# farhad-dalirani/StereoVision-SLAM

Hardware: AMD Instinct MI355X
Metric: stereo frames/sec (track + local BA), KITTI-00-shaped synthetic stereo 1241x376 (620x188 after the reference's 1/2 decimation) (higher is better)
Workload: dtype u8/i32 fixed-point (pyramid, LK), f32 (GFTT), f64 (LM, BA)

## Files before the change

stereovision-slam_amd/csrc/k_lk.h:

```cpp
#pragma once
#include "dev_common.h"

struct LkJob { int prev_slot, next_slot, pt_ofs, npts; };
struct LkParams {
    int max_level;
    int max_count;
    double eps2;
    double min_eig_thr;
    int use_initial_flow;
    float eig_num_thr;
    int eig_use_div;
    int njobs, blocks_per_job;
};

#define LK_WIN 11
#define LK_NPIX 121
#define LK_W_BITS 14
#define LK_REG 32
#ifndef LK_WAVES_PER_BLOCK
#define LK_WAVES_PER_BLOCK 1
#endif
#define LK_IROW 20

typedef uint32_t lk_u32_ua __attribute__((aligned(1)));
typedef uint16_t lk_u16_ua __attribute__((aligned(1)));
typedef short lk_s2 __attribute__((ext_vector_type(2)));

__device__ __forceinline__ int lk_dot2(uint32_t a, uint32_t b, int c)
{
    int r;
    asm("v_dot2_i32_i16 %0, %1, %2, %3" : "=v"(r) : "v"(a), "v"(b), "v"(c));
    return r;
}
#define LK_PAIR_SEL0 0x0c010c00u
__device__ __forceinline__ uint32_t lk_pair_sel(int a) { return LK_PAIR_SEL0 + (uint32_t)(a & 3) * 0x00010001u; }
__device__ __forceinline__ uint32_t lk_pair_at(const uint32_t *base32, int a, uint32_t sel)
{
    const uint32_t *q = base32 + (a >> 2);
    return __builtin_amdgcn_perm(q[1], q[0], sel);
}

__device__ __forceinline__ int lk_floor_i(float x)
{
    int r;
    asm("v_cvt_flr_i32_f32 %0, %1" : "=v"(r) : "v"(x));
    return r;
}

struct LkW { uint32_t top, bot; };

__device__ __forceinline__ LkW lk_weights(float a, float b)
{
    typedef float lk_f2 __attribute__((ext_vector_type(2)));
    const float S = (float)(1 << LK_W_BITS), M = 12582912.f;
    const float A = a * S, An = S - A, bn = 1.f - b;
    const lk_f2 p0 = (lk_f2){An, A} * (lk_f2){bn, bn} + (lk_f2){M, M};
    const uint32_t b00 = __float_as_uint(p0.x), b01 = __float_as_uint(p0.y), b10 = __float_as_uint(An * b + M);
    const uint32_t w11 = ((1u << LK_W_BITS) + 3u * 0x4B400000u) - (b00 + b01 + b10);
    LkW w;
    w.top = __builtin_amdgcn_perm(b01, b00, 0x05040100u);
    w.bot = __builtin_amdgcn_perm(w11, b10, 0x05040100u);
    return w;
}

__device__ __forceinline__ int lk_sample_u8(const uint32_t *base32, int a, int row_stride, LkW w)
{
    const uint32_t sel = lk_pair_sel(a);
    const uint32_t *q = base32 + (a >> 2);
    const int rs = row_stride >> 2;
    const uint32_t t = __builtin_amdgcn_perm(q[1], q[0], sel), b = __builtin_amdgcn_perm(q[rs + 1], q[rs], sel);
    return lk_dot2(t, w.top, lk_dot2(b, w.bot, 1 << (LK_W_BITS - 5 - 1))) >> (LK_W_BITS - 5);
}

__device__ __forceinline__ int lk_sample_diff(const uint32_t *base32, int a, int row_stride, LkW w, int acc0)
{
    const uint32_t sel = lk_pair_sel(a);
    const uint32_t *q = base32 + (a >> 2);
    const int rs = row_stride >> 2;
    const uint32_t t = __builtin_amdgcn_perm(q[1], q[0], sel), b = __builtin_amdgcn_perm(q[rs + 1], q[rs], sel);
    return lk_dot2(t, w.top, lk_dot2(b, w.bot, acc0)) >> (LK_W_BITS - 5);
}

typedef const __attribute__((address_space(3))) uint32_t *lk_lds_u32;
__device__ __forceinline__ int lk_sample_diff_at(uint32_t addr, LkW w, int acc0)
{
    lk_lds_u32 q = (lk_lds_u32)(uintptr_t)addr;
    const uint32_t t = q[0], b = q[LK_REG];
    return lk_dot2(t, w.top, lk_dot2(b, w.bot, acc0)) >> (LK_W_BITS - 5);
}

struct LkJRegs { uint32_t v[4]; };
__device__ __forceinline__ LkJRegs lk_stage_J_issue(const uint8_t *J0, uint32_t lofs, int pitch, int w, int h,
                                                    int cx, int cy, int lane, int &rx0, int &ry0)
{
    rx0 = __builtin_amdgcn_readfirstlane((cx - 10) & ~3);
    ry0 = __builtin_amdgcn_readfirstlane(cy - 10);
    const int r = lane >> 3, c4 = lane & 7;
    LkJRegs o;
    if (rx0 >= -SVS_BORDER && rx0 + LK_REG <= w + SVS_BORDER && ry0 >= -SVS_BORDER && ry0 + LK_REG <= h + SVS_BORDER) {
        const uint32_t p = lofs + (uint32_t)((ry0 + r) * pitch + (rx0 + c4 * 4));
#pragma unroll
        for (int k = 0; k < 4; ++k)
            o.v[k] = *reinterpret_cast<const uint32_t *>(J0 + (p + (uint32_t)(8 * k * pitch)));
    } else {
        const int gxmax = (w + SVS_BORDER - 4) & ~3;
        const int gx = max(-SVS_BORDER, min(rx0 + c4 * 4, gxmax));
#pragma unroll
        for (int k = 0; k < 4; ++k) {
            const int gy = max(-SVS_BORDER, min(ry0 + r + 8 * k, h + SVS_BORDER - 1));
            o.v[k] = *reinterpret_cast<const uint32_t *>(J0 + (lofs + (uint32_t)(gy * pitch + gx)));
        }
    }
    return o;
}
__device__ __forceinline__ void lk_stage_J_commit(uint32_t *sJ, const LkJRegs &o, int lane)
{
    typedef uint32_t lk_u4 __attribute__((ext_vector_type(4)));
    const int r = lane >> 3, c4 = lane & 7;
#pragma unroll
    for (int k = 0; k < 4; ++k) {
        const uint32_t cur = o.v[k];
        const uint32_t nxt = (uint32_t)__builtin_amdgcn_update_dpp(0, (int)cur, 0x101 , 0xf, 0xf, true);
        lk_u4 pr;
        pr.x = __builtin_amdgcn_perm(nxt, cur, 0x0c010c00u);
        pr.y = __builtin_amdgcn_perm(nxt, cur, 0x0c020c01u);
        pr.z = __builtin_amdgcn_perm(nxt, cur, 0x0c030c02u);
        pr.w = __builtin_amdgcn_perm(nxt, cur, 0x0c040c03u);
        *reinterpret_cast<lk_u4 *>(sJ + (r + 8 * k) * LK_REG + 4 * c4) = pr;
    }
    __builtin_amdgcn_fence(__ATOMIC_RELEASE, "wavefront");
    __builtin_amdgcn_wave_barrier();
}
__device__ __forceinline__ void lk_stage_J(uint32_t *sJ, const uint8_t *J0, uint32_t lofs, int pitch, int w, int h,
                                           int cx, int cy, int lane, int &rx0, int &ry0)
{
    const LkJRegs o = lk_stage_J_issue(J0, lofs, pitch, w, h, cx, cy, lane, rx0, ry0);
    lk_stage_J_commit(sJ, o, lane);
}

__device__ __forceinline__ float lk_sum_to_f32(long long s, float scale)
{
    const int lo = (int)s;
    const bool fits = (long long)lo == s;
    const int t = fits ? lo : (int)((s >> 1) | (s & 1));
    const uint32_t kb = fits ? __float_as_uint(scale) : __float_as_uint(2.f * scale);
    return (float)t * __uint_as_float(kb);
}

typedef unsigned lk_u2 __attribute__((ext_vector_type(2)));
__device__ __forceinline__ int lk_row_reduce(int w)
{
    w += dpp_i32<SVS_DPP_XOR1>(w);
    w += dpp_i32<SVS_DPP_XOR2>(w);
    w += dpp_i32<SVS_DPP_HALF_MIRROR>(w);
    w += dpp_i32<SVS_DPP_MIRROR>(w);
    return w;
}
__device__ __forceinline__ void lk_wave_sum2_i32(int a, int b, int &sa, int &sb)
{
    const lk_u2 r = __builtin_amdgcn_permlane16_swap((unsigned)a, (unsigned)b, false, false);
    const int v = (int)(r.x + r.y);
    const int w = lk_row_reduce(v);
    sa = __builtin_amdgcn_readlane(w, 0) + __builtin_amdgcn_readlane(w, 32);
    sb = __builtin_amdgcn_readlane(w, 16) + __builtin_amdgcn_readlane(w, 48);
}
__device__ __forceinline__ void lk_wave_sum4_i32(int a, int b, int c, int d, int &sa, int &sb, int &sc, int &sd)
{
    const lk_u2 r1 = __builtin_amdgcn_permlane16_swap((unsigned)a, (unsigned)b, false, false);
    const lk_u2 r2 = __builtin_amdgcn_permlane16_swap((unsigned)c, (unsigned)d, false, false);
    const int v1 = (int)(r1.x + r1.y), v2 = (int)(r2.x + r2.y);
    const lk_u2 q = __builtin_amdgcn_permlane32_swap((unsigned)v1, (unsigned)v2, false, false);
    const int w = lk_row_reduce((int)(q.x + q.y));
    sa = __builtin_amdgcn_readlane(w, 0);
    sb = __builtin_amdgcn_readlane(w, 16);
    sc = __builtin_amdgcn_readlane(w, 32);
    sd = __builtin_amdgcn_readlane(w, 48);
}

#ifndef LK_OCC_TEST
#define LK_OCC_TEST 0
#endif
#if LK_OCC_TEST == 1
#define LK_OCC_ATTR __attribute__((amdgpu_waves_per_eu(8, 8)))
#else
#define LK_OCC_ATTR
#endif
__global__ void __launch_bounds__(64 * LK_WAVES_PER_BLOCK) LK_OCC_ATTR
k_lk(const LkJob *jobs, const uint8_t *pyr, PyrGeom g, const float2 *prev_xy, float2 *next_xy,
     uint8_t *status, float *err, LkParams prm)
{
    __shared__ uint32_t sI_all[LK_WAVES_PER_BLOCK][16 * LK_IROW / 4 + 2];
    __shared__ uint32_t sD_all[LK_WAVES_PER_BLOCK][144];
    __shared__ __attribute__((aligned(16))) uint32_t sJ_all[LK_WAVES_PER_BLOCK][LK_REG * LK_REG];

#if LK_OCC_TEST == 2
    __shared__ uint32_t sPad[8192];
    sPad[threadIdx.x] = threadIdx.x;
    if (prm.max_count < 0) status[0] = (uint8_t)sPad[(threadIdx.x * 37) & 8191];
#endif
    const int wave = threadIdx.x >> 6, lane = threadIdx.x & 63;
    const int slot = blockIdx.x >> 3, round = slot / prm.blocks_per_job;
    const int job = round * 8 + (blockIdx.x & 7);
    if (job >= prm.njobs) return;
    const LkJob jb = jobs[job];
    const int pi = (slot - round * prm.blocks_per_job) * LK_WAVES_PER_BLOCK + wave;
    if (pi >= jb.npts) return;
    const int pt = jb.pt_ofs + pi;
    uint32_t *sI32 = sI_all[wave];
    uint32_t *sD = sD_all[wave];
    uint32_t *sJ = sJ_all[wave];

    const uint8_t *slotI = pyr + (size_t)jb.prev_slot * g.slot_bytes;
    const uint8_t *slotJ = pyr + (size_t)jb.next_slot * g.slot_bytes;

    const float2 prevp = prev_xy[pt];
    float2 nextp = next_xy[pt];
    bool st = true;
    float errv = 0.f;

    const int p0 = lane, p1 = lane + 64;
    const bool has1 = p1 < LK_NPIX;
    const int wy0 = p0 / LK_WIN, wx0 = p0 - wy0 * LK_WIN;
    const int wy1 = has1 ? p1 / LK_WIN : 0, wx1 = has1 ? p1 - wy1 * LK_WIN : 0;
    const int oI0 = (wy0 + 1) * LK_IROW + wx0 + 1, oI1 = (wy1 + 1) * LK_IROW + wx1 + 1;
    const int oD0 = wy0 * 12 + wx0, oD1 = wy1 * 12 + wx1;
    const int oJ0 = wy0 * LK_REG + wx0, oJ1 = wy1 * LK_REG + wx1;
    const uint32_t aJ0 = (uint32_t)(uintptr_t)(__attribute__((address_space(3))) uint32_t *)sJ + 4u * (uint32_t)oJ0,
                   aJ1 = (uint32_t)(uintptr_t)(__attribute__((address_space(3))) uint32_t *)sJ + 4u * (uint32_t)oJ1;
    const int sr = lane >> 2, sc = (lane & 3) * 3;
    const float FLT_SCALE = 1.f / (float)(1 << 20);
    const float e_lo = (float)(prm.eps2 * (1.0 - 2e-6)), e_hi = (float)(prm.eps2 * (1.0 + 2e-6));

    int max_level = prm.max_level;
    if (max_level > g.nlevels - 1) max_level = g.nlevels - 1;

    for (int level = max_level; level >= 0; --level) {
        const int w = g.w[level], h = g.h[level], pitch = g.pitch[level];
        const uint32_t lofs = (uint32_t)g.ofs[level] + (uint32_t)(SVS_BORDER * pitch + SVS_BORDER);
        const float lscale = __uint_as_float((uint32_t)(127 - level) << 23);
        float px = prevp.x * lscale, py = prevp.y * lscale;
        float nx, ny;
        if (level == max_level) {
            if (prm.use_initial_flow) { nx = nextp.x * lscale; ny = nextp.y * lscale; }
            else { nx = px; ny = py; }
        } else { nx = nextp.x * 2.f; ny = nextp.y * 2.f; }
        nextp.x = nx; nextp.y = ny;

        px -= 5.f; py -= 5.f;
        const int ipx = __builtin_amdgcn_readfirstlane(lk_floor_i(px)), ipy = __builtin_amdgcn_readfirstlane(lk_floor_i(py));
        const uint32_t wext = (uint32_t)(w + LK_WIN), hext = (uint32_t)(h + LK_WIN);
        if ((uint32_t)(ipx + LK_WIN) >= wext || (uint32_t)(ipy + LK_WIN) >= hext) {
            if (level == 0) { st = false; errv = 0.f; }
            continue;
        }
        const LkW iw = lk_weights(px - (float)ipx, py - (float)ipy);

        const int xs = (ipx - 1) & ~3, a0 = (ipx - 1) & 3;
        __builtin_amdgcn_wave_barrier();
        nx -= 5.f; ny -= 5.f;
        int rx0, ry0;
        LkJRegs jr;
        {
            const uint32_t ib = lofs + (uint32_t)((ipy - 1) * pitch + xs);
            const uint32_t v0 = *reinterpret_cast<const uint32_t *>(slotI + (ib + (uint32_t)((lane >> 2) * pitch + (lane & 3) * 4)));
            const uint32_t v1 = *reinterpret_cast<const uint32_t *>(slotI + (ib + (uint32_t)((lane & 15) * pitch + 16)));
            jr = lk_stage_J_issue(slotJ, lofs, pitch, w, h, lk_floor_i(nx), lk_floor_i(ny), lane, rx0, ry0);
            sI32[(lane >> 2) * (LK_IROW / 4) + (lane & 3)] = v0;
            sI32[(lane & 15) * (LK_IROW / 4) + 4] = v1;
        }
        __builtin_amdgcn_fence(__ATOMIC_RELEASE, "wavefront");
        __builtin_amdgcn_wave_barrier();
        if (lane < 48) {
            const int ab = sr * LK_IROW + a0 + sc;
            const int k8 = (ab & 3) * 8;
            const uint32_t *q = sI32 + (ab >> 2);
            const uint32_t al = q[0], ah = q[1], bl = q[LK_IROW / 4], bh = q[LK_IROW / 4 + 1],
                           cl = q[2 * (LK_IROW / 4)], ch = q[2 * (LK_IROW / 4) + 1];
            const uint32_t a4 = __builtin_amdgcn_alignbyte(ah, al, ab & 3), b4 = __builtin_amdgcn_alignbyte(bh, bl, ab & 3),
                           c4 = __builtin_amdgcn_alignbyte(ch, cl, ab & 3);
            auto pr = [](uint32_t v) -> lk_s2 { return __builtin_bit_cast(lk_s2, v); };
            const lk_s2 A01 = pr(__builtin_amdgcn_perm(0u, a4, 0x0c010c00u)), A23 = pr(__builtin_amdgcn_perm(0u, a4, 0x0c030c02u)), A4 = pr((ah >> k8) & 0xffu);
            const lk_s2 B01 = pr(__builtin_amdgcn_perm(0u, b4, 0x0c010c00u)), B23 = pr(__builtin_amdgcn_perm(0u, b4, 0x0c030c02u)), B4 = pr((bh >> k8) & 0xffu);
            const lk_s2 C01 = pr(__builtin_amdgcn_perm(0u, c4, 0x0c010c00u)), C23 = pr(__builtin_amdgcn_perm(0u, c4, 0x0c030c02u)), C4 = pr((ch >> k8) & 0xffu);
            const lk_s2 k3 = { 3, 3 }, k10 = { 10, 10 };
            const lk_s2 T001 = (A01 + C01) * k3 + B01 * k10, T023 = (A23 + C23) * k3 + B23 * k10, T04 = (A4 + C4) * k3 + B4 * k10;
            const lk_s2 T101 = C01 - A01, T123 = C23 - A23, T14 = C4 - A4;
            const lk_s2 DX01 = T023 - T001, DX2 = T04 - T023;
            const lk_s2 M01 = pr(__builtin_amdgcn_alignbyte(__builtin_bit_cast(uint32_t, T123), __builtin_bit_cast(uint32_t, T101), 2));
            const lk_s2 M2 = pr(__builtin_amdgcn_alignbyte(__builtin_bit_cast(uint32_t, T14), __builtin_bit_cast(uint32_t, T123), 2));
            const lk_s2 DY01 = (T123 + T101) * k3 + M01 * k10, DY2 = (T14 + T123) * k3 + M2 * k10;
            const uint32_t dx01 = __builtin_bit_cast(uint32_t, DX01), dy01 = __builtin_bit_cast(uint32_t, DY01);
            const uint32_t o0 = __builtin_amdgcn_perm(dy01, dx01, 0x05040100u), o1 = __builtin_amdgcn_perm(dy01, dx01, 0x07060302u),
                           o2 = __builtin_amdgcn_perm(__builtin_bit_cast(uint32_t, DY2), __builtin_bit_cast(uint32_t, DX2), 0x05040100u);
            const bool rowin = (uint32_t)(ipy + sr) < (uint32_t)h;
            sD[sr * 12 + sc + 0] = o0 & (0u - (uint32_t)(rowin & ((uint32_t)(ipx + sc + 0) < (uint32_t)w)));
            sD[sr * 12 + sc + 1] = o1 & (0u - (uint32_t)(rowin & ((uint32_t)(ipx + sc + 1) < (uint32_t)w)));
            sD[sr * 12 + sc + 2] = o2 & (0u - (uint32_t)(rowin & ((uint32_t)(ipx + sc + 2) < (uint32_t)w)));
        }
        __builtin_amdgcn_fence(__ATOMIC_RELEASE, "wavefront");
        __builtin_amdgcn_wave_barrier();
        int iv0, ix0, iy0, iv1, ix1, iy1;
        {
            iv0 = lk_sample_u8(sI32, oI0 + a0, LK_IROW, iw);
            const uint32_t d00 = sD[oD0], d01 = sD[oD0 + 1], d10 = sD[oD0 + 12], d11 = sD[oD0 + 13];
            ix0 = lk_dot2(__builtin_amdgcn_perm(d01, d00, 0x05040100u), iw.top,
                          lk_dot2(__builtin_amdgcn_perm(d11, d10, 0x05040100u), iw.bot, 1 << (LK_W_BITS - 1))) >> LK_W_BITS;
            iy0 = lk_dot2(__builtin_amdgcn_perm(d01, d00, 0x07060302u), iw.top,
                          lk_dot2(__builtin_amdgcn_perm(d11, d10, 0x07060302u), iw.bot, 1 << (LK_W_BITS - 1))) >> LK_W_BITS;
        }
        {
            iv1 = lk_sample_u8(sI32, oI1 + a0, LK_IROW, iw);
            const uint32_t d00 = sD[oD1], d01 = sD[oD1 + 1], d10 = sD[oD1 + 12], d11 = sD[oD1 + 13];
            ix1 = lk_dot2(__builtin_amdgcn_perm(d01, d00, 0x05040100u), iw.top,
                          lk_dot2(__builtin_amdgcn_perm(d11, d10, 0x05040100u), iw.bot, 1 << (LK_W_BITS - 1))) >> LK_W_BITS;
            iy1 = lk_dot2(__builtin_amdgcn_perm(d01, d00, 0x07060302u), iw.top,
                          lk_dot2(__builtin_amdgcn_perm(d11, d10, 0x07060302u), iw.bot, 1 << (LK_W_BITS - 1))) >> LK_W_BITS;
            if (!has1) { ix1 = 0; iy1 = 0; }
        }
        int sA11, sA12, sA22, sIdle;
        lk_wave_sum4_i32(__mul24(ix0, ix0) + __mul24(ix1, ix1), __mul24(ix0, iy0) + __mul24(ix1, iy1), __mul24(iy0, iy0) + __mul24(iy1, iy1), 0,
                         sA11, sA12, sA22, sIdle);
        const float A11 = (float)sA11 * FLT_SCALE, A12 = (float)sA12 * FLT_SCALE, A22 = (float)sA22 * FLT_SCALE;
        float D = A11 * A22 - A12 * A12;
        const float dd = A11 - A22;
        const float q2 = dd * dd + 4.f * A12 * A12;
        float eigNum;
        if (prm.eig_use_div) eigNum = A22 + A11 - sqrtf(q2);
        else {
            const float sq = __builtin_amdgcn_sqrtf(q2);
            eigNum = A22 + A11 - sq;
            if (fabsf(eigNum - prm.eig_num_thr) <= sq * 4.8e-7f + 1e-30f) eigNum = A22 + A11 - sqrtf(q2);
        }
        const bool eigSmall = prm.eig_use_div ? (double)(eigNum / (float)(2 * LK_WIN * LK_WIN)) < prm.min_eig_thr : eigNum < prm.eig_num_thr;
        if (eigSmall || D < 1.1920928955078125e-07f) {
            if (level == 0) st = false;
            continue;
        }
        D = 1.f / D;
        const bool narrow = sA11 <= 570000000 && sA22 <= 570000000;
        const int acc00 = (1 << (LK_W_BITS - 5 - 1)) - (iv0 << (LK_W_BITS - 5)), acc01 = (1 << (LK_W_BITS - 5 - 1)) - (iv1 << (LK_W_BITS - 5));
        const uint32_t ixx = __builtin_amdgcn_perm((uint32_t)ix1, (uint32_t)ix0, 0x05040100u), iyy = __builtin_amdgcn_perm((uint32_t)iy1, (uint32_t)iy0, 0x05040100u);
        float pdx = 0.f, pdy = 0.f, dx = 0.f, dy = 0.f;
        const float Ds = D * FLT_SCALE;
        bool moved = false, osc = false;
        lk_stage_J_commit(sJ, jr, lane);

        for (int j = 0; j < prm.max_count; ++j) {
            const int inx = __builtin_amdgcn_readfirstlane(lk_floor_i(nx)), iny = __builtin_amdgcn_readfirstlane(lk_floor_i(ny));
            if ((uint32_t)(inx + LK_WIN) >= wext || (uint32_t)(iny + LK_WIN) >= hext) {
                if (level == 0) st = false;
                break;
            }
            int ox = inx - rx0, oy = iny - ry0;
            if ((uint32_t)ox > LK_REG - 12 || (uint32_t)oy > LK_REG - 12) {
                lk_stage_J(sJ, slotJ, lofs, pitch, w, h, inx, iny, lane, rx0, ry0);
                ox = inx - rx0; oy = iny - ry0;
            }
            const LkW jw = lk_weights(nx - (float)inx, ny - (float)iny);
            const uint32_t jo = 4u * (uint32_t)(oy * LK_REG + ox);
            const int d0 = lk_sample_diff_at(aJ0 + jo, jw, acc00);
            const int d1 = lk_sample_diff_at(aJ1 + jo, jw, acc01);
            const uint32_t dd01 = __builtin_amdgcn_perm((uint32_t)d1, (uint32_t)d0, 0x05040100u);
            const int pb1 = lk_dot2(dd01, ixx, 0), pb2 = lk_dot2(dd01, iyy, 0);
            float b1, b2;
            if (narrow) {
                int s1, s2;
                lk_wave_sum2_i32(pb1, pb2, s1, s2);
                b1 = (float)s1; b2 = (float)s2;
            } else {
                b1 = lk_sum_to_f32(wave_sum_i32_wide(pb1), 1.f); b2 = lk_sum_to_f32(wave_sum_i32_wide(pb2), 1.f);
            }
            dx = (A12 * b2 - A22 * b1) * Ds;
            dy = (A12 * b1 - A11 * b2) * Ds;
            nx += dx; ny += dy;
            moved = true;
            const float dd2 = dx * dx + dy * dy;
            if (dd2 < e_lo) break;
            if (dd2 <= e_hi && (double)dx * (double)dx + (double)dy * (double)dy <= prm.eps2) break;
            if (j > 0 && fabsf(dx + pdx) <= 0.01f && fabsf(dy + pdy) <= 0.01f) {
                osc = true;
                break;
            }
            pdx = dx; pdy = dy;
        }
        if (moved) {
            nextp.x = nx + 5.f; nextp.y = ny + 5.f;
            if (osc) { nextp.x -= dx * 0.5f; nextp.y -= dy * 0.5f; }
        }

        if (st && level == 0) {
            const float fx = nextp.x - 5.f, fy = nextp.y - 5.f;
            const int inx = __builtin_amdgcn_readfirstlane(lk_floor_i(fx)), iny = __builtin_amdgcn_readfirstlane(lk_floor_i(fy));
            if (inx < -LK_WIN || inx >= w || iny < -LK_WIN || iny >= h) {
                st = false;
                continue;
            }
            int ox = inx - rx0, oy = iny - ry0;
            if (ox < 0 || ox > LK_REG - 12 || oy < 0 || oy > LK_REG - 12) {
                lk_stage_J(sJ, slotJ, lofs, pitch, w, h, inx, iny, lane, rx0, ry0);
                ox = inx - rx0; oy = iny - ry0;
            }
            const LkW jw = lk_weights(fx - (float)inx, fy - (float)iny);
            const uint32_t jo = 4u * (uint32_t)(oy * LK_REG + ox);
            const int d0 = lk_sample_diff_at(aJ0 + jo, jw, 1 << (LK_W_BITS - 5 - 1)) - iv0;
            const int d1 = lk_sample_diff_at(aJ1 + jo, jw, 1 << (LK_W_BITS - 5 - 1)) - iv1;
            const int e = (d0 < 0 ? -d0 : d0) + (has1 ? (d1 < 0 ? -d1 : d1) : 0);
            const int serr = wave_sum_i32(e);
            errv = (float)serr * 1.f / (float)(32 * LK_WIN * LK_WIN);
        }
    }
    if (lane == 0) {
        next_xy[pt] = nextp;
        status[pt] = st ? 1 : 0;
        if (err) err[pt] = errv;
    }
}
```

Measured before the change: 588,400.

## Compute all pyramid levels' LK template setup in parallel, one 16-lane row per level

The per-level template setup (I-window load, Scharr gradients, bilinear sampling, structure-tensor reduction) that used to run serially at each pyramid level inside the coarse-to-fine loop is now done once up front. Each 16-lane row of the wave handles one level. The results are handed over through LDS that aliases the J region, plus registers for the coarse levels, and the iteration loop just reads them. This removes the serial global-load latency and barriers paid at every level. In exchange it uses more registers, does 4x redundant lane work per row, and ties the code to SVS_LEVELS==4.

```diff
diff --git a/stereovision-slam_amd/csrc/k_lk.h b/stereovision-slam_amd/csrc/k_lk.h
--- a/stereovision-slam_amd/csrc/k_lk.h
+++ b/stereovision-slam_amd/csrc/k_lk.h
@@ -21,6 +21,9 @@
 #define LK_WAVES_PER_BLOCK 1
 #endif
 #define LK_IROW 20
+#define LK_SI_DW (16 * LK_IROW / 4 + 2)
+#define LK_SETUP_DW (LK_SI_DW + 144)
+#define LK_SCAL_DW 8
 
 typedef uint32_t lk_u32_ua __attribute__((aligned(1)));
 typedef uint16_t lk_u16_ua __attribute__((aligned(1)));
@@ -164,17 +167,9 @@
     sa = __builtin_amdgcn_readlane(w, 0) + __builtin_amdgcn_readlane(w, 32);
     sb = __builtin_amdgcn_readlane(w, 16) + __builtin_amdgcn_readlane(w, 48);
 }
-__device__ __forceinline__ void lk_wave_sum4_i32(int a, int b, int c, int d, int &sa, int &sb, int &sc, int &sd)
-{
-    const lk_u2 r1 = __builtin_amdgcn_permlane16_swap((unsigned)a, (unsigned)b, false, false);
-    const lk_u2 r2 = __builtin_amdgcn_permlane16_swap((unsigned)c, (unsigned)d, false, false);
-    const int v1 = (int)(r1.x + r1.y), v2 = (int)(r2.x + r2.y);
-    const lk_u2 q = __builtin_amdgcn_permlane32_swap((unsigned)v1, (unsigned)v2, false, false);
-    const int w = lk_row_reduce((int)(q.x + q.y));
-    sa = __builtin_amdgcn_readlane(w, 0);
-    sb = __builtin_amdgcn_readlane(w, 16);
-    sc = __builtin_amdgcn_readlane(w, 32);
-    sd = __builtin_amdgcn_readlane(w, 48);
+__device__ __forceinline__ float lk_uniform_f32(uint32_t v)
+{
+    return __uint_as_float((uint32_t)__builtin_amdgcn_readfirstlane((int)v));
 }
 
 #ifndef LK_OCC_TEST
@@ -189,9 +184,11 @@
 k_lk(const LkJob *jobs, const uint8_t *pyr, PyrGeom g, const float2 *prev_xy, float2 *next_xy,
      uint8_t *status, float *err, LkParams prm)
 {
-    __shared__ uint32_t sI_all[LK_WAVES_PER_BLOCK][16 * LK_IROW / 4 + 2];
-    __shared__ uint32_t sD_all[LK_WAVES_PER_BLOCK][144];
     __shared__ __attribute__((aligned(16))) uint32_t sJ_all[LK_WAVES_PER_BLOCK][LK_REG * LK_REG];
+    __shared__ uint32_t sH_all[LK_WAVES_PER_BLOCK][3 * 64 + SVS_LEVELS * LK_SCAL_DW];
+    static_assert(SVS_LEVELS == 4, "one 16-lane row per pyramid level, three coarse levels held in registers");
+    static_assert(SVS_LEVELS * LK_SETUP_DW <= LK_REG * LK_REG && (SVS_LEVELS - 1) * 3 * 64 <= LK_REG * LK_REG,
+                  "the set-up scratch and the coarse levels' hand-over alias the J region");
 
 #if LK_OCC_TEST == 2
     __shared__ uint32_t sPad[8192];
@@ -206,9 +203,8 @@
     const int pi = (slot - round * prm.blocks_per_job) * LK_WAVES_PER_BLOCK + wave;
     if (pi >= jb.npts) return;
     const int pt = jb.pt_ofs + pi;
-    uint32_t *sI32 = sI_all[wave];
-    uint32_t *sD = sD_all[wave];
     uint32_t *sJ = sJ_all[wave];
+    uint32_t *sH = sH_all[wave];
 
     const uint8_t *slotI = pyr + (size_t)jb.prev_slot * g.slot_bytes;
     const uint8_t *slotJ = pyr + (size_t)jb.next_slot * g.slot_bytes;
@@ -222,106 +218,110 @@
     const bool has1 = p1 < LK_NPIX;
     const int wy0 = p0 / LK_WIN, wx0 = p0 - wy0 * LK_WIN;
     const int wy1 = has1 ? p1 / LK_WIN : 0, wx1 = has1 ? p1 - wy1 * LK_WIN : 0;
-    const int oI0 = (wy0 + 1) * LK_IROW + wx0 + 1, oI1 = (wy1 + 1) * LK_IROW + wx1 + 1;
-    const int oD0 = wy0 * 12 + wx0, oD1 = wy1 * 12 + wx1;
     const int oJ0 = wy0 * LK_REG + wx0, oJ1 = wy1 * LK_REG + wx1;
     const uint32_t aJ0 = (uint32_t)(uintptr_t)(__attribute__((address_space(3))) uint32_t *)sJ + 4u * (uint32_t)oJ0,
                    aJ1 = (uint32_t)(uintptr_t)(__attribute__((address_space(3))) uint32_t *)sJ + 4u * (uint32_t)oJ1;
-    const int sr = lane >> 2, sc = (lane & 3) * 3;
     const float FLT_SCALE = 1.f / (float)(1 << 20);
     const float e_lo = (float)(prm.eps2 * (1.0 - 2e-6)), e_hi = (float)(prm.eps2 * (1.0 + 2e-6));
 
     int max_level = prm.max_level;
     if (max_level > g.nlevels - 1) max_level = g.nlevels - 1;
 
-    for (int level = max_level; level >= 0; --level) {
-        const int w = g.w[level], h = g.h[level], pitch = g.pitch[level];
-        const uint32_t lofs = (uint32_t)g.ofs[level] + (uint32_t)(SVS_BORDER * pitch + SVS_BORDER);
-        const float lscale = __uint_as_float((uint32_t)(127 - level) << 23);
+    uint32_t *sS = sH + 3 * 64;
+    uint32_t hc[SVS_LEVELS - 1][3];
+    {
+        const int row = lane >> 4, rl = lane & 15;
+        const int lev = min(row, max_level);
+        int w = g.w[0], h = g.h[0], pitch = g.pitch[0];
+        uint32_t ofs = (uint32_t)g.ofs[0];
+#pragma unroll
+        for (int l = 1; l < SVS_LEVELS; ++l)
+            if (lev == l) { w = g.w[l]; h = g.h[l]; pitch = g.pitch[l]; ofs = (uint32_t)g.ofs[l]; }
+        const uint32_t lofs = ofs + (uint32_t)(SVS_BORDER * pitch + SVS_BORDER);
+        const float lscale = __uint_as_float((uint32_t)(127 - lev) << 23);
         float px = prevp.x * lscale, py = prevp.y * lscale;
-        float nx, ny;
-        if (level == max_level) {
-            if (prm.use_initial_flow) { nx = nextp.x * lscale; ny = nextp.y * lscale; }
-            else { nx = px; ny = py; }
-        } else { nx = nextp.x * 2.f; ny = nextp.y * 2.f; }
-        nextp.x = nx; nextp.y = ny;
-
         px -= 5.f; py -= 5.f;
-        const int ipx = __builtin_amdgcn_readfirstlane(lk_floor_i(px)), ipy = __builtin_amdgcn_readfirstlane(lk_floor_i(py));
-        const uint32_t wext = (uint32_t)(w + LK_WIN), hext = (uint32_t)(h + LK_WIN);
-        if ((uint32_t)(ipx + LK_WIN) >= wext || (uint32_t)(ipy + LK_WIN) >= hext) {
-            if (level == 0) { st = false; errv = 0.f; }
-            continue;
-        }
+        int ipx = lk_floor_i(px), ipy = lk_floor_i(py);
+        const bool outside = (uint32_t)(ipx + LK_WIN) >= (uint32_t)(w + LK_WIN) || (uint32_t)(ipy + LK_WIN) >= (uint32_t)(h + LK_WIN);
+        if (outside) { ipx = 0; ipy = 0; }
         const LkW iw = lk_weights(px - (float)ipx, py - (float)ipy);
+        uint32_t *sI32 = sJ + row * LK_SETUP_DW, *sD = sI32 + LK_SI_DW;
 
         const int xs = (ipx - 1) & ~3, a0 = (ipx - 1) & 3;
-        __builtin_amdgcn_wave_barrier();
-        nx -= 5.f; ny -= 5.f;
-        int rx0, ry0;
-        LkJRegs jr;
         {
-            const uint32_t ib = lofs + (uint32_t)((ipy - 1) * pitch + xs);
-            const uint32_t v0 = *reinterpret_cast<const uint32_t *>(slotI + (ib + (uint32_t)((lane >> 2) * pitch + (lane & 3) * 4)));
-            const uint32_t v1 = *reinterpret_cast<const uint32_t *>(slotI + (ib + (uint32_t)((lane & 15) * pitch + 16)));
-            jr = lk_stage_J_issue(slotJ, lofs, pitch, w, h, lk_floor_i(nx), lk_floor_i(ny), lane, rx0, ry0);
-            sI32[(lane >> 2) * (LK_IROW / 4) + (lane & 3)] = v0;
-            sI32[(lane & 15) * (LK_IROW / 4) + 4] = v1;
+            const uint32_t ib = lofs + (uint32_t)((ipy - 1 + rl) * pitch + xs);
+            uint32_t v[LK_IROW / 4];
+#pragma unroll
+            for (int k = 0; k < LK_IROW / 4; ++k) v[k] = *reinterpret_cast<const uint32_t *>(slotI + (ib + 4u * k));
+#pragma unroll
+            for (int k = 0; k < LK_IROW / 4; ++k) sI32[rl * (LK_IROW / 4) + k] = v[k];
         }
         __builtin_amdgcn_fence(__ATOMIC_RELEASE, "wavefront");
         __builtin_amdgcn_wave_barrier();
-        if (lane < 48) {
-            const int ab = sr * LK_IROW + a0 + sc;
-            const int k8 = (ab & 3) * 8;
-            const uint32_t *q = sI32 + (ab >> 2);
-            const uint32_t al = q[0], ah = q[1], bl = q[LK_IROW / 4], bh = q[LK_IROW / 4 + 1],
-                           cl = q[2 * (LK_IROW / 4)], ch = q[2 * (LK_IROW / 4) + 1];
-            const uint32_t a4 = __builtin_amdgcn_alignbyte(ah, al, ab & 3), b4 = __builtin_amdgcn_alignbyte(bh, bl, ab & 3),
-                           c4 = __builtin_amdgcn_alignbyte(ch, cl, ab & 3);
-            auto pr = [](uint32_t v) -> lk_s2 { return __builtin_bit_cast(lk_s2, v); };
-            const lk_s2 A01 = pr(__builtin_amdgcn_perm(0u, a4, 0x0c010c00u)), A23 = pr(__builtin_amdgcn_perm(0u, a4, 0x0c030c02u)), A4 = pr((ah >> k8) & 0xffu);
-            const lk_s2 B01 = pr(__builtin_amdgcn_perm(0u, b4, 0x0c010c00u)), B23 = pr(__builtin_amdgcn_perm(0u, b4, 0x0c030c02u)), B4 = pr((bh >> k8) & 0xffu);
-            const lk_s2 C01 = pr(__builtin_amdgcn_perm(0u, c4, 0x0c010c00u)), C23 = pr(__builtin_amdgcn_perm(0u, c4, 0x0c030c02u)), C4 = pr((ch >> k8) & 0xffu);
-            const lk_s2 k3 = { 3, 3 }, k10 = { 10, 10 };
-            const lk_s2 T001 = (A01 + C01) * k3 + B01 * k10, T023 = (A23 + C23) * k3 + B23 * k10, T04 = (A4 + C4) * k3 + B4 * k10;
-            const lk_s2 T101 = C01 - A01, T123 = C23 - A23, T14 = C4 - A4;
-            const lk_s2 DX01 = T023 - T001, DX2 = T04 - T023;
-            const lk_s2 M01 = pr(__builtin_amdgcn_alignbyte(__builtin_bit_cast(uint32_t, T123), __builtin_bit_cast(uint32_t, T101), 2));
-            const lk_s2 M2 = pr(__builtin_amdgcn_alignbyte(__builtin_bit_cast(uint32_t, T14), __builtin_bit_cast(uint32_t, T123), 2));
-            const lk_s2 DY01 = (T123 + T101) * k3 + M01 * k10, DY2 = (T14 + T123) * k3 + M2 * k10;
-            const uint32_t dx01 = __builtin_bit_cast(uint32_t, DX01), dy01 = __builtin_bit_cast(uint32_t, DY01);
-            const uint32_t o0 = __builtin_amdgcn_perm(dy01, dx01, 0x05040100u), o1 = __builtin_amdgcn_perm(dy01, dx01, 0x07060302u),
-                           o2 = __builtin_amdgcn_perm(__builtin_bit_cast(uint32_t, DY2), __builtin_bit_cast(uint32_t, DX2), 0x05040100u);
-            const bool rowin = (uint32_t)(ipy + sr) < (uint32_t)h;
-            sD[sr * 12 + sc + 0] = o0 & (0u - (uint32_t)(rowin & ((uint32_t)(ipx + sc + 0) < (uint32_t)w)));
-            sD[sr * 12 + sc + 1] = o1 & (0u - (uint32_t)(rowin & ((uint32_t)(ipx + sc + 1) < (uint32_t)w)));
-            sD[sr * 12 + sc + 2] = o2 & (0u - (uint32_t)(rowin & ((uint32_t)(ipx + sc + 2) < (uint32_t)w)));
+        {
+            const int sc = (rl & 3) * 3;
+            const int sh = (a0 + sc) & 3, k8 = sh * 8;
+            const uint32_t m0 = 0u - (uint32_t)((uint32_t)(ipx + sc + 0) < (uint32_t)w), m1 = 0u - (uint32_t)((uint32_t)(ipx + sc + 1) < (uint32_t)w),
+                           m2 = 0u - (uint32_t)((uint32_t)(ipx + sc + 2) < (uint32_t)w);
+#pragma unroll
+            for (int k = 0; k < 3; ++k) {
+                const int sr = (rl >> 2) + 4 * k;
+                const int ab = sr * LK_IROW + a0 + sc;
+                const uint32_t *q = sI32 + (ab >> 2);
+                const uint32_t al = q[0], ah = q[1], bl = q[LK_IROW / 4], bh = q[LK_IROW / 4 + 1],
+                               cl = q[2 * (LK_IROW / 4)], ch = q[2 * (LK_IROW / 4) + 1];
+                const uint32_t a4 = __builtin_amdgcn_alignbyte(ah, al, sh), b4 = __builtin_amdgcn_alignbyte(bh, bl, sh),
+                               c4 = __builtin_amdgcn_alignbyte(ch, cl, sh);
+                auto pr = [](uint32_t v) -> lk_s2 { return __builtin_bit_cast(lk_s2, v); };
+                const lk_s2 A01 = pr(__builtin_amdgcn_perm(0u, a4, 0x0c010c00u)), A23 = pr(__builtin_amdgcn_perm(0u, a4, 0x0c030c02u)), A4 = pr((ah >> k8) & 0xffu);
+                const lk_s2 B01 = pr(__builtin_amdgcn_perm(0u, b4, 0x0c010c00u)), B23 = pr(__builtin_amdgcn_perm(0u, b4, 0x0c030c02u)), B4 = pr((bh >> k8) & 0xffu);
+                const lk_s2 C01 = pr(__builtin_amdgcn_perm(0u, c4, 0x0c010c00u)), C23 = pr(__builtin_amdgcn_perm(0u, c4, 0x0c030c02u)), C4 = pr((ch >> k8) & 0xffu);
+                const lk_s2 k3 = { 3, 3 }, k10 = { 10, 10 };
+                const lk_s2 T001 = (A01 + C01) * k3 + B01 * k10, T023 = (A23 + C23) * k3 + B23 * k10, T04 = (A4 + C4) * k3 + B4 * k10;
+                const lk_s2 T101 = C01 - A01, T123 = C23 - A23, T14 = C4 - A4;
+                const lk_s2 DX01 = T023 - T001, DX2 = T04 - T023;
+                const lk_s2 M01 = pr(__builtin_amdgcn_alignbyte(__builtin_bit_cast(uint32_t, T123), __builtin_bit_cast(uint32_t, T101), 2));
+                const lk_s2 M2 = pr(__builtin_amdgcn_alignbyte(__builtin_bit_cast(uint32_t, T14), __builtin_bit_cast(uint32_t, T123), 2));
+                const lk_s2 DY01 = (T123 + T101) * k3 + M01 * k10, DY2 = (T14 + T123) * k3 + M2 * k10;
+                const uint32_t dx01 = __builtin_bit_cast(uint32_t, DX01), dy01 = __builtin_bit_cast(uint32_t, DY01);
+                const uint32_t o0 = __builtin_amdgcn_perm(dy01, dx01, 0x05040100u), o1 = __builtin_amdgcn_perm(dy01, dx01, 0x07060302u),
+                               o2 = __builtin_amdgcn_perm(__builtin_bit_cast(uint32_t, DY2), __builtin_bit_cast(uint32_t, DX2), 0x05040100u);
+                const uint32_t rowin = 0u - (uint32_t)((uint32_t)(ipy + sr) < (uint32_t)h);
+                sD[sr * 12 + sc + 0] = o0 & rowin & m0;
+                sD[sr * 12 + sc + 1] = o1 & rowin & m1;
+                sD[sr * 12 + sc + 2] = o2 & rowin & m2;
+            }
         }
         __builtin_amdgcn_fence(__ATOMIC_RELEASE, "wavefront");
         __builtin_amdgcn_wave_barrier();
-        int iv0, ix0, iy0, iv1, ix1, iy1;
-        {
-            iv0 = lk_sample_u8(sI32, oI0 + a0, LK_IROW, iw);
-            const uint32_t d00 = sD[oD0], d01 = sD[oD0 + 1], d10 = sD[oD0 + 12], d11 = sD[oD0 + 13];
-            ix0 = lk_dot2(__builtin_amdgcn_perm(d01, d00, 0x05040100u), iw.top,
-                          lk_dot2(__builtin_amdgcn_perm(d11, d10, 0x05040100u), iw.bot, 1 << (LK_W_BITS - 1))) >> LK_W_BITS;
-            iy0 = lk_dot2(__builtin_amdgcn_perm(d01, d00, 0x07060302u), iw.top,
-                          lk_dot2(__builtin_amdgcn_perm(d11, d10, 0x07060302u), iw.bot, 1 << (LK_W_BITS - 1))) >> LK_W_BITS;
-        }
-        {
-            iv1 = lk_sample_u8(sI32, oI1 + a0, LK_IROW, iw);
-            const uint32_t d00 = sD[oD1], d01 = sD[oD1 + 1], d10 = sD[oD1 + 12], d11 = sD[oD1 + 13];
-            ix1 = lk_dot2(__builtin_amdgcn_perm(d01, d00, 0x05040100u), iw.top,
-                          lk_dot2(__builtin_amdgcn_perm(d11, d10, 0x05040100u), iw.bot, 1 << (LK_W_BITS - 1))) >> LK_W_BITS;
-            iy1 = lk_dot2(__builtin_amdgcn_perm(d01, d00, 0x07060302u), iw.top,
-                          lk_dot2(__builtin_amdgcn_perm(d11, d10, 0x07060302u), iw.bot, 1 << (LK_W_BITS - 1))) >> LK_W_BITS;
-            if (!has1) { ix1 = 0; iy1 = 0; }
-        }
-        int sA11, sA12, sA22, sIdle;
-        lk_wave_sum4_i32(__mul24(ix0, ix0) + __mul24(ix1, ix1), __mul24(ix0, iy0) + __mul24(ix1, iy1), __mul24(iy0, iy0) + __mul24(iy1, iy1), 0,
-                         sA11, sA12, sA22, sIdle);
+        int a11 = 0, a12 = 0, a22 = 0;
+        uint32_t hv[4][3];
+#pragma unroll
+        for (int m = 0; m < 4; ++m) {
+            const int l = rl + 16 * m;
+            int iv[2], ix[2], iy[2];
+#pragma unroll
+            for (int s = 0; s < 2; ++s) {
+                const int p = l + 64 * s;
+                const bool has = s == 0 || p < LK_NPIX;
+                const int wy = has ? p / LK_WIN : 0, wx = has ? p - wy * LK_WIN : 0;
+                const int oI = (wy + 1) * LK_IROW + wx + 1, oD = wy * 12 + wx;
+                iv[s] = lk_sample_u8(sI32, oI + a0, LK_IROW, iw);
+                const uint32_t d00 = sD[oD], d01 = sD[oD + 1], d10 = sD[oD + 12], d11 = sD[oD + 13];
+                ix[s] = lk_dot2(__builtin_amdgcn_perm(d01, d00, 0x05040100u), iw.top,
+                                lk_dot2(__builtin_amdgcn_perm(d11, d10, 0x05040100u), iw.bot, 1 << (LK_W_BITS - 1))) >> LK_W_BITS;
+                iy[s] = lk_dot2(__builtin_amdgcn_perm(d01, d00, 0x07060302u), iw.top,
+                                lk_dot2(__builtin_amdgcn_perm(d11, d10, 0x07060302u), iw.bot, 1 << (LK_W_BITS - 1))) >> LK_W_BITS;
+                if (!has) { ix[s] = 0; iy[s] = 0; }
+                a11 += __mul24(ix[s], ix[s]); a12 += __mul24(ix[s], iy[s]); a22 += __mul24(iy[s], iy[s]);
+            }
+            hv[m][0] = __builtin_amdgcn_perm((uint32_t)iv[1], (uint32_t)iv[0], 0x05040100u);
+            hv[m][1] = __builtin_amdgcn_perm((uint32_t)ix[1], (uint32_t)ix[0], 0x05040100u);
+            hv[m][2] = __builtin_amdgcn_perm((uint32_t)iy[1], (uint32_t)iy[0], 0x05040100u);
+        }
+        const int sA11 = lk_row_reduce(a11), sA12 = lk_row_reduce(a12), sA22 = lk_row_reduce(a22);
         const float A11 = (float)sA11 * FLT_SCALE, A12 = (float)sA12 * FLT_SCALE, A22 = (float)sA22 * FLT_SCALE;
-        float D = A11 * A22 - A12 * A12;
+        const float D = A11 * A22 - A12 * A12;
         const float dd = A11 - A22;
         const float q2 = dd * dd + 4.f * A12 * A12;
         float eigNum;
@@ -332,16 +332,65 @@
             if (fabsf(eigNum - prm.eig_num_thr) <= sq * 4.8e-7f + 1e-30f) eigNum = A22 + A11 - sqrtf(q2);
         }
         const bool eigSmall = prm.eig_use_div ? (double)(eigNum / (float)(2 * LK_WIN * LK_WIN)) < prm.min_eig_thr : eigNum < prm.eig_num_thr;
-        if (eigSmall || D < 1.1920928955078125e-07f) {
-            if (level == 0) st = false;
+        const bool narrow = sA11 <= 570000000 && sA22 <= 570000000;
+        const uint32_t flags = (outside ? 1u : 0u) | ((eigSmall || D < 1.1920928955078125e-07f) ? 2u : 0u) | (narrow ? 4u : 0u);
+        __builtin_amdgcn_fence(__ATOMIC_RELEASE, "wavefront");
+        __builtin_amdgcn_wave_barrier();
+        uint32_t *sHl = row == 0 ? sH : sJ + (row - 1) * (3 * 64);
+#pragma unroll
+        for (int m = 0; m < 4; ++m) {
+            sHl[rl + 16 * m] = hv[m][0];
+            sHl[64 + rl + 16 * m] = hv[m][1];
+            sHl[128 + rl + 16 * m] = hv[m][2];
+        }
+        if (rl == 0) {
+            uint32_t *s = sS + row * LK_SCAL_DW;
+            s[0] = __float_as_uint(A11); s[1] = __float_as_uint(A12); s[2] = __float_as_uint(A22);
+            s[3] = __float_as_uint((1.f / D) * FLT_SCALE); s[4] = flags;
+        }
+        __builtin_amdgcn_fence(__ATOMIC_RELEASE, "wavefront");
+        __builtin_amdgcn_wave_barrier();
+#pragma unroll
+        for (int l = 0; l < SVS_LEVELS - 1; ++l)
+#pragma unroll
+            for (int k = 0; k < 3; ++k) hc[l][k] = sJ[l * (3 * 64) + k * 64 + lane];
+    }
+    __builtin_amdgcn_fence(__ATOMIC_RELEASE, "wavefront");
+    __builtin_amdgcn_wave_barrier();
+
+    for (int level = max_level; level >= 0; --level) {
+        const int w = g.w[level], h = g.h[level], pitch = g.pitch[level];
+        const uint32_t lofs = (uint32_t)g.ofs[level] + (uint32_t)(SVS_BORDER * pitch + SVS_BORDER);
+        const float lscale = __uint_as_float((uint32_t)(127 - level) << 23);
+        float nx, ny;
+        if (level == max_level) {
+            if (prm.use_initial_flow) { nx = nextp.x * lscale; ny = nextp.y * lscale; }
+            else { nx = prevp.x * lscale; ny = prevp.y * lscale; }
+        } else { nx = nextp.x * 2.f; ny = nextp.y * 2.f; }
+        nextp.x = nx; nextp.y = ny;
+
+        const uint32_t *sSl = sS + level * LK_SCAL_DW;
+        const uint32_t flags = __builtin_amdgcn_readfirstlane(sSl[4]);
+        if (flags & 3) {
+            if (level == 0) { st = false; errv = 0.f; }
             continue;
         }
-        D = 1.f / D;
-        const bool narrow = sA11 <= 570000000 && sA22 <= 570000000;
+        const uint32_t wext = (uint32_t)(w + LK_WIN), hext = (uint32_t)(h + LK_WIN);
+        nx -= 5.f; ny -= 5.f;
+        int rx0, ry0;
+        const LkJRegs jr = lk_stage_J_issue(slotJ, lofs, pitch, w, h, lk_floor_i(nx), lk_floor_i(ny), lane, rx0, ry0);
+        const float A11 = lk_uniform_f32(sSl[0]), A12 = lk_uniform_f32(sSl[1]), A22 = lk_uniform_f32(sSl[2]), Ds = lk_uniform_f32(sSl[3]);
+        const bool narrow = (flags & 4) != 0;
+        uint32_t ivv, ixx, iyy;
+        if (level == 0) { ivv = sH[lane]; ixx = sH[64 + lane]; iyy = sH[128 + lane]; }
+        else {
+            ivv = level == 1 ? hc[0][0] : level == 2 ? hc[1][0] : hc[2][0];
+            ixx = level == 1 ? hc[0][1] : level == 2 ? hc[1][1] : hc[2][1];
+            iyy = level == 1 ? hc[0][2] : level == 2 ? hc[1][2] : hc[2][2];
+        }
+        const int iv0 = (int)(ivv & 0xffffu), iv1 = (int)(ivv >> 16);
         const int acc00 = (1 << (LK_W_BITS - 5 - 1)) - (iv0 << (LK_W_BITS - 5)), acc01 = (1 << (LK_W_BITS - 5 - 1)) - (iv1 << (LK_W_BITS - 5));
-        const uint32_t ixx = __builtin_amdgcn_perm((uint32_t)ix1, (uint32_t)ix0, 0x05040100u), iyy = __builtin_amdgcn_perm((uint32_t)iy1, (uint32_t)iy0, 0x05040100u);
         float pdx = 0.f, pdy = 0.f, dx = 0.f, dy = 0.f;
-        const float Ds = D * FLT_SCALE;
         bool moved = false, osc = false;
         lk_stage_J_commit(sJ, jr, lane);
 
```

New measurement: 608,100 (median of 5 runs). +3.4%, better.
